# Mattdl/CLsurvey

Hardware: AMD Instinct MI355X
Metric: images/sec (train+importance pass), EWC small_VGG9 Tiny-ImageNet task batch (higher is better)
Workload: dtype f32 (bf16x6 split operands on the conv fwd/bwd-data matrix products, fp32 accumulate); 1 GPU; EWC small_VGG9_cl_128_128, Tiny-ImageNet shapes (3x64x64, 20 classes), batch 200: train step + Fisher step (BASELINE configs[1]); batch=200, parallelism=1 GPU

## Files before the change

clsurvey_amd/csrc/bsconv.hip:

```cpp
#include "common.hpp"
#include "bs_weight.hpp"
#include "wgrad_reduce.hpp"
#include <cstdlib>

#ifndef BS_ABL
#define BS_ABL 0
#endif

namespace {

constexpr int BS_WT_JOBS = 24;
struct BsWtJobs { int n; int pad; clhip_wino_wt j[BS_WT_JOBS]; int first[BS_WT_JOBS + 1]; };

__global__ __launch_bounds__(256) void bs_weight_multi_kernel(BsWtJobs J) {
    int jb = 0;
    for (int i = 1; i < J.n; ++i) jb = ((int)blockIdx.x >= J.first[i]) ? i : jb;
    bs_weight_block(J.j[jb], (int)blockIdx.x - J.first[jb], (int)threadIdx.x);
}

template <int RW_, int RH_, int NI_, int WAVES_M_, int WM_, int WN_, int KS_ = 3>
struct BsGeo {
    static constexpr int RW = RW_, RH = RH_, NI = NI_, WAVES_M = WAVES_M_, WAVES_N = 4 / WAVES_M_, WM = WM_, WN = WN_;
    static constexpr int KS = KS_, HP = KS_ / 2, TAPS = KS_ * KS_;
    static constexpr int BM = RW * RH * NI;
    static_assert(BM == 32 * WAVES_M * WM, "pixels per block = M tiles of the waves");
    static_assert(32 * WAVES_N * WN == BS_BN, "64 output channels per block");
    static constexpr int MTW = RW >= 16 ? 16 : 8, MTH = 32 / MTW;
    static_assert(RW % MTW == 0 && RH % MTH == 0, "whole M tiles");
    static constexpr int MT_PER_ROW = RW / MTW, MT_PER_IMG = MT_PER_ROW * (RH / MTH);
    static constexpr int IPR = RW == 8 ? 2 : 1;
    static_assert(NI % IPR == 0, "image pairs");
    static constexpr int HW_ = RW + 2 * HP, HR = RH + 2 * HP;
    static constexpr int P = (IPR * HW_ + 7) / 16 * 16 + 8;
    static_assert(P >= IPR * HW_ && P % 16 == 8, "pitch");
    static constexpr int ROWS = (NI / IPR) * HR;
    static constexpr int PLANE_SLOTS = (ROWS - 1) * P + IPR * HW_;
    static constexpr int PLANE_BYTES = PLANE_SLOTS * 16;
    static constexpr int BUF_BYTES = 6 * PLANE_BYTES;
    static constexpr int NHALO = NI * HR * HW_;
    static constexpr int ITEMS = 2 * NHALO;
    static constexpr int ROUNDS = (ITEMS + 255) / 256;
    static_assert(ROUNDS * 256 - ITEMS <= ITEMS, "the last round wraps at most once");
    static constexpr int TPR = WM < MT_PER_ROW ? WM : MT_PER_ROW;
    static_assert(WM % TPR == 0 && MT_PER_ROW % TPR == 0 && MT_PER_IMG % WM == 0, "a wave's tiles form a rectangle inside one image");
    static constexpr int RGW = TPR * MTW, RGH = 32 * WM / RGW;
    static constexpr int TS = 32 * WM + 4;
    static_assert(4 * 32 * TS * 4 <= 2 * BUF_BYTES, "transposition buffers fit the staging LDS");
};

template <class G, int MODE, bool UNPOOL>
__device__ __forceinline__ void bs_conv_body(
    unsigned char* __restrict__ lds, const int b, const float* __restrict__ in, const clhip_u32x4* __restrict__ wimg,
    const float* __restrict__ bias, const float* __restrict__ mask_src, float* __restrict__ out, uint8_t* __restrict__ pool_idx, int N,
    int Cin, int Cout, int H, int W, int relu, int tiles_x, int tiles_y, int npb) {
    constexpr int RW = G::RW, RH = G::RH, NI = G::NI, WM = G::WM, WN = G::WN, P = G::P, HR = G::HR, HW_ = G::HW_;
    constexpr int ROUNDS = G::ROUNDS;

    const int tid = threadIdx.x, lane = tid & 63, wave = tid >> 6;
    const int kts = (Cout + BS_BN - 1) / BS_BN;
    const int kt = (b >> 3) % kts, pb = (b / (8 * kts)) * 8 + (b & 7);
    if (pb >= npb) return;
    const int tx = pb % tiles_x, ty = (pb / tiles_x) % tiles_y, grp = pb / (tiles_x * tiles_y);
    const int n0 = grp * NI, y0 = ty * RH, x0 = tx * RW;
    const int n_chunks = Cin / BS_CK;
    const int IH = UNPOOL ? H >> 1 : H, IW = UNPOOL ? W >> 1 : W;
    const int plane_in = IH * IW;

    const float* in_blk = in + (size_t)n0 * Cin * plane_in;
    const __amdgpu_buffer_rsrc_t rs_x = clhip_rsrc(in_blk, (size_t)(N - n0) * Cin * plane_in * sizeof(float));
    const __amdgpu_buffer_rsrc_t rs_i = clhip_rsrc(UNPOOL ? pool_idx + (size_t)n0 * Cin * plane_in : pool_idx,
                                                   UNPOOL ? (size_t)(N - n0) * Cin * plane_in : 0);
    const int n_nt = (Cout + 31) / 32;
    constexpr int TAPS = G::TAPS, KS = G::KS;
    const __amdgpu_buffer_rsrc_t rs_w = clhip_rsrc(wimg, (size_t)n_nt * n_chunks * 3 * TAPS * 1024);

    int xoff[ROUNDS], lw[ROUNDS], pos[ROUNDS];
#pragma unroll
    for (int r = 0; r < ROUNDS; ++r) {
        const int it_ = r * 256 + tid, it = it_ < G::ITEMS ? it_ : it_ - G::ITEMS;
        const int h = it >= G::NHALO ? 1 : 0, p = it - h * G::NHALO;
        const int ni = p / (HR * HW_), rem = p - ni * (HR * HW_), hy = rem / HW_, hx = rem - hy * HW_;
        const int gy = y0 + hy - G::HP, gx = x0 + hx - G::HP, n = n0 + ni;
        const bool ok = n < N && gy >= 0 && gy < H && gx >= 0 && gx < W;
        const int e = UNPOOL ? (gy >> 1) * IW + (gx >> 1) : gy * IW + gx;
        xoff[r] = ok ? (ni * Cin + 8 * h) * plane_in + e : CLHIP_OOB;
        pos[r] = ((gy & 1) << 1) | (gx & 1);
        lw[r] = (h * G::PLANE_SLOTS + ((ni / G::IPR) * HR + hy) * P + (ni % G::IPR) * HW_ + hx) * 16;
    }
    float xr[ROUNDS][8];
    unsigned xi[UNPOOL ? ROUNDS : 1][8];
    auto load_chunk = [&](int c) {
        if (BS_ABL & 8) return;
        const int cb = c * BS_CK * plane_in;
#pragma unroll
        for (int r = 0; r < ROUNDS; ++r)
#pragma unroll
            for (int e = 0; e < 8; ++e) {
                const int so = cb + e * plane_in;
                xr[r][e] = clhip_buf_load(rs_x, xoff[r] != CLHIP_OOB ? xoff[r] * 4 : CLHIP_OOB, so * 4);
                if constexpr (UNPOOL) xi[r][e] = clhip_buf_load_u8(rs_i, xoff[r], so);
            }
    };
    auto store_chunk = [&](int buf) {
        if (BS_ABL & 4) return;
#pragma unroll
        for (int r = 0; r < ROUNDS; ++r) {
            float v[8];
#pragma unroll
            for (int e = 0; e < 8; ++e) {
                if constexpr (UNPOOL) v[e] = xi[r][e] == (unsigned)pos[r] ? xr[r][e] : 0.f;
                else v[e] = xr[r][e];
            }
            clhip_u32x4 q0, q1, q2;
            bs_split8(v, q0, q1, q2);
            unsigned char* d = lds + buf * G::BUF_BYTES + lw[r];
            *reinterpret_cast<clhip_u32x4*>(d) = q0;
            *reinterpret_cast<clhip_u32x4*>(d + 2 * G::PLANE_BYTES) = q1;
            *reinterpret_cast<clhip_u32x4*>(d + 4 * G::PLANE_BYTES) = q2;
        }
    };

    const int wm = wave % G::WAVES_M, wn = wave / G::WAVES_M;
    const int m = lane & 31, kh = lane >> 5;
    const int mw = m >> 2, mq = m & 3;
    const int prow = 2 * (mw / (G::MTW / 2)) + (mq >> 1), pcol = 2 * (mw % (G::MTW / 2)) + (mq & 1);
    int abase[WM];
#pragma unroll
    for (int i = 0; i < WM; ++i) {
        const int mt = wm * WM + i;
        const int ni = mt / G::MT_PER_IMG, rem = mt - ni * G::MT_PER_IMG, tr = rem / G::MT_PER_ROW, tc = rem - tr * G::MT_PER_ROW;
        abase[i] = (kh * G::PLANE_SLOTS + ((ni / G::IPR) * HR + tr * G::MTH + prow) * P + (ni % G::IPR) * HW_ + tc * G::MTW + pcol) * 16;
    }
    const int nt0 = kt * (BS_BN / 32) + wn * WN;
    int wvoff[WN];
#pragma unroll
    for (int j = 0; j < WN; ++j) wvoff[j] = (nt0 + j < n_nt) ? ((nt0 + j) * n_chunks * 3 * TAPS * 64 + lane) * 16 : CLHIP_OOB;
    auto load_b = [&](clhip_u32x4 (&bq)[WN][3], int c, int tap) {
        if (BS_ABL & 2) return;
        const int so = (c * 3 * TAPS + tap * 3) * 1024;
#pragma unroll
        for (int j = 0; j < WN; ++j)
#pragma unroll
            for (int s = 0; s < 3; ++s) bq[j][s] = __builtin_amdgcn_raw_buffer_load_b128(rs_w, wvoff[j], so + s * 1024, 0);
    };

    floatx16 acc[WM][WN], accl[WM][WN];
#pragma unroll
    for (int i = 0; i < WM; ++i)
#pragma unroll
        for (int j = 0; j < WN; ++j)
#pragma unroll
            for (int r = 0; r < 16; ++r) {
// ... 186 lines not shown
                    }
                }
                if (!ok || ((BS_ABL & 16) && y00 != 12345.678f)) continue;
                const size_t o = ((size_t)n * Cout + k) * chw + (size_t)oh * W + ow;
                if (odd) {
                    const bool row1 = oh + 1 < H, col1 = ow + 1 < W;
                    if (MODE == 1 && mask_src) {
                        y00 = mask_src[o] > 0.f ? y00 : 0.f;
                        if (col1) y01 = mask_src[o + 1] > 0.f ? y01 : 0.f;
                        if (row1) y10 = mask_src[o + W] > 0.f ? y10 : 0.f;
                        if (row1 && col1) y11 = mask_src[o + W + 1] > 0.f ? y11 : 0.f;
                    }
                    out[o] = y00;
                    if (col1) out[o + 1] = y01;
                    if (row1) out[o + W] = y10;
                    if (row1 && col1) out[o + W + 1] = y11;
                } else {
                    if (MODE == 1 && mask_src) {
                        const float2 m0 = *reinterpret_cast<const float2*>(mask_src + o), m1 = *reinterpret_cast<const float2*>(mask_src + o + W);
                        y00 = m0.x > 0.f ? y00 : 0.f; y01 = m0.y > 0.f ? y01 : 0.f;
                        y10 = m1.x > 0.f ? y10 : 0.f; y11 = m1.y > 0.f ? y11 : 0.f;
                    }
                    *reinterpret_cast<float2*>(out + o) = make_float2(y00, y01);
                    *reinterpret_cast<float2*>(out + o + W) = make_float2(y10, y11);
                }
            }
        }
    }
    }
}

template <class G, bool UNPOOL>
constexpr int bs_blocks_per_cu() {
    return (3 * 2 * G::BUF_BYTES <= 160 * 1024 && (G::RW == 32 || (!UNPOOL && G::KS == 3))) ? 3 : 2;
}

template <class G, int MODE, bool UNPOOL>
__global__ __launch_bounds__(256, (bs_blocks_per_cu<G, UNPOOL>())) void bs_conv_kernel(
    const float* __restrict__ in, const clhip_u32x4* __restrict__ wimg, const float* __restrict__ bias,
    const float* __restrict__ mask_src, float* __restrict__ out, uint8_t* __restrict__ pool_idx, int N, int Cin, int Cout, int H,
    int W, int relu, int tiles_x, int tiles_y, int npb) {
    __shared__ __attribute__((aligned(16))) unsigned char lds[2 * G::BUF_BYTES];
    bs_conv_body<G, MODE, UNPOOL>(lds, (int)blockIdx.x, in, wimg, bias, mask_src, out, pool_idx, N, Cin, Cout, H, W, relu, tiles_x, tiles_y, npb);
}

template <class GA, class GB, int MODE, bool UNPOOL>
__global__ __launch_bounds__(256, (bs_blocks_per_cu<GA, UNPOOL>() < bs_blocks_per_cu<GB, UNPOOL>() ? bs_blocks_per_cu<GA, UNPOOL>()
                                                                                                  : bs_blocks_per_cu<GB, UNPOOL>()))
void bs_conv_mixed_kernel(const float* __restrict__ in, const clhip_u32x4* __restrict__ wimg, const float* __restrict__ bias,
                          const float* __restrict__ mask_src, float* __restrict__ out, uint8_t* __restrict__ pool_idx, int N, int Cin,
                          int Cout, int H, int W, int relu, int blocks_a, int NA, int tiles_xa, int tiles_ya, int npb_a, int tiles_xb,
                          int tiles_yb, int npb_b) {
    constexpr int LB = 2 * (GA::BUF_BYTES > GB::BUF_BYTES ? GA::BUF_BYTES : GB::BUF_BYTES);
    __shared__ __attribute__((aligned(16))) unsigned char lds[LB];
    const int b = (int)blockIdx.x;
    if (b < blocks_a) {
        bs_conv_body<GA, MODE, UNPOOL>(lds, b, in, wimg, bias, mask_src, out, pool_idx, NA, Cin, Cout, H, W, relu, tiles_xa, tiles_ya, npb_a);
    } else {
        const size_t in_img = (size_t)Cin * (UNPOOL ? (size_t)(H >> 1) * (W >> 1) : (size_t)H * W);
        const bool pool = MODE == 0 && pool_idx != nullptr;
        const size_t out_img = (size_t)Cout * (pool ? (size_t)(H >> 1) * (W >> 1) : (size_t)H * W);
        uint8_t* idx_b = pool_idx ? pool_idx + (size_t)NA * (UNPOOL ? in_img : out_img) : nullptr;
        bs_conv_body<GB, MODE, UNPOOL>(lds, b - blocks_a, in + (size_t)NA * in_img, wimg, bias,
                                       mask_src ? mask_src + (size_t)NA * Cout * H * W : nullptr, out + (size_t)NA * out_img, idx_b, N - NA,
                                       Cin, Cout, H, W, relu, tiles_xb, tiles_yb, npb_b);
    }
}
// ... 134 lines not shown
BsMixed bs_one_geo(int N, int Cout, int H, int W) {
    BsMixed m{};
    m.txa = (W + G::RW - 1) / G::RW; m.tya = (H + G::RH - 1) / G::RH; m.NA = N;
    const long long npb = (long long)m.txa * m.tya * ((N + G::NI - 1) / G::NI);
    const long long blocks = (npb + 7) / 8 * 8 * ((Cout + BS_BN - 1) / BS_BN);
    m.blocks = (npb > 0x7fffffffLL || blocks > 0x7fffffffLL) ? 0 : blocks;
    m.npb_a = (int)npb; m.blocks_a = (int)m.blocks;
    return m;
}

template <bool UNPOOL>
int bs_launch_riders(const float* in, const clhip_u32x4* wimg, const float* mask_src, float* out, uint8_t* pool_idx, int N, int Cin,
                     int Cout, int H, int W, const RedJobs& jobs, int place, int riders, hipStream_t s) {
#define BS_RIDE(GA_, GB_, M_) return bs_launch_riders_geo<GA_, GB_, UNPOOL>(in, wimg, mask_src, out, pool_idx, N, Cin, Cout, H, W, M_, jobs, place, riders, s)
    if (W > 16 && !((H | W) & 1)) {
        BsMixed m;
        if (bs_mixed32_plan<UNPOOL>(N, Cout, H, W, m)) BS_RIDE(BsGA32, BsGB32, m);
    }
    using G16 = BsGeo<16, 8, 1, 2, 2, 1>;
    using G8 = BsGeo<8, 8, 2, 2, 2, 1>;
    if (W > 16) BS_RIDE(BsGA32, BsGA32, bs_one_geo<BsGA32>(N, Cout, H, W));
    if (W > 8) BS_RIDE(G16, G16, bs_one_geo<G16>(N, Cout, H, W));
    BS_RIDE(G8, G8, bs_one_geo<G8>(N, Cout, H, W));
#undef BS_RIDE
}

template <int MODE>
int bs_launch5(const float* in, const clhip_u32x4* wimg, const float* bias, const float* mask_src, float* out, int N, int Cin, int Cout,
               int H, int W, int relu, hipStream_t s) {
    if (W > 16) return bs_launch_geo<BsGeo<32, 4, 1, 2, 2, 1, 5>, MODE, false>(in, wimg, bias, mask_src, out, nullptr, N, Cin, Cout, H, W, relu, s);
    return bs_launch_geo<BsGeo<16, 8, 1, 2, 2, 1, 5>, MODE, false>(in, wimg, bias, mask_src, out, nullptr, N, Cin, Cout, H, W, relu, s);
}

}

bool clhip_internal_bs_ok(int Cin, int Cout, int H, int W) {
    return Cin >= 32 && Cin % 32 == 0 && Cout >= 64 && Cout % 64 == 0 && H >= 4 && W >= 4;
}

bool clhip_internal_bs_index_ok(int Cin, int Cout, int H, int W, int ks) {
    const long long px = (long long)H * W, ni = (ks == 3 && W <= 8) ? 2 : 1;
    const long long img = (long long)((Cout + 31) / 32) * ((Cin + BS_CK - 1) / BS_CK) * 3 * ks * ks * 1024;
    return ni * Cin * px < (1LL << 29) && Cout * px < (1LL << 29) && img <= 0x7fffffffLL;
}

bool clhip_internal_bs_preferred(int Cin, int Cout, int H, int W) {
    static const int mode = bs_env_int("CLHIP_BS", 1);
    if (mode == 0 || !clhip_internal_bs_ok(Cin, Cout, H, W)) return false;
    if (mode == 2) return true;
    const long long px = (long long)H * W;
    return (px >= 1024 && px <= 4096 && Cin <= 128 && Cout <= 128) || (px >= 512 && px < 1024 && Cin >= 256 && Cout >= 256);
}
bool clhip_internal_bs5_preferred(int Cin, int Cout, int H, int W) {
    static const int mode = bs_env_int("CLHIP_BS", 1);
    return mode != 0 && clhip_internal_bs_ok(Cin, Cout, H, W) && W > 8;
}

size_t clhip_internal_bs_ws(int Cin, int Cout) {
    return (size_t)((Cout + 31) / 32) * ((Cin + BS_CK - 1) / BS_CK) * 27 * 1024;
}
size_t clhip_internal_bs5_ws(int Cin, int Cout) {
    return (size_t)((Cout + 31) / 32) * ((Cin + BS_CK - 1) / BS_CK) * 75 * 1024;
}

int clhip_internal_bs_weights(const clhip_wino_wt* jobs, int n, hipStream_t s) {
    if (n <= 0) return 0;
// ... 110 lines not shown
    if (N <= 0 || !clhip_internal_bs_ok(K, C, H, W)) return CLHIP_ENOTSUP;
    if (!dy || !w || !dx || !ws || ws_bytes < clhip_internal_bs_ws(K, C)) return CLHIP_EINVAL;
    if (!clhip_internal_bs_index_ok(K, C, H, W, 3)) return CLHIP_EINVAL;
    if (((H | W) & 1) && idx_u8_or_null) return CLHIP_ENOTSUP;
    const clhip_wino_wt job{w, static_cast<float*>(ws), C, K, 1, 0};
    const int rc = clhip_internal_bs_weights(&job, 1, as_stream(stream));
    if (rc) return rc;
    return clhip_internal_bs_conv_u(1, dy, ws, nullptr, relu_src, dx, const_cast<uint8_t*>(idx_u8_or_null), idx_u8_or_null != nullptr,
                                    N, K, C, H, W, 0, as_stream(stream));
}

int clhip_conv3x3_bs_bwd_data_riders(const float* dy, const uint8_t* idx_u8_or_null, const float* w, const float* relu_src, float* dx, int N,
                                     int C, int K, int H, int W, void* ws, size_t ws_bytes, const clhip_reduce_job* jobs, int n_jobs,
                                     int place, int riders, void* stream) {
    if (N <= 0 || !clhip_internal_bs_ok(K, C, H, W)) return CLHIP_ENOTSUP;
    if (!dy || !w || !dx || !ws || ws_bytes < clhip_internal_bs_ws(K, C)) return CLHIP_EINVAL;
    if (!clhip_internal_bs_index_ok(K, C, H, W, 3)) return CLHIP_EINVAL;
    if (((H | W) & 1) && idx_u8_or_null) return CLHIP_ENOTSUP;
    if (!jobs || n_jobs < 1 || n_jobs > CLHIP_WGRAD_JOBS_MAX || place < 1 || place > 3 || riders < 8 || riders % 8 || riders > (1 << 20))
        return CLHIP_ENOTSUP;
    clhip_wgrad_job q[CLHIP_WGRAD_JOBS_MAX];
    for (int i = 0; i < n_jobs; ++i) {
        const clhip_reduce_job& j = jobs[i];
        if (!j.slabs || !j.dw || j.K <= 0 || j.C <= 0 || j.splits <= 0 || (j.taps != 9 && j.taps != 25)) return CLHIP_EINVAL;
        q[i] = clhip_wgrad_job{j.slabs, j.dw, j.db, j.K, j.C, j.splits, j.taps};
    }
    const clhip_wino_wt job{w, static_cast<float*>(ws), C, K, 1, 0};
    const int rc = clhip_internal_bs_weights(&job, 1, as_stream(stream));
    if (rc) return rc;
    return clhip_internal_bs_conv_u_riders(dy, ws, relu_src, dx, const_cast<uint8_t*>(idx_u8_or_null), idx_u8_or_null != nullptr, N, K, C, H,
                                           W, q, n_jobs, place, riders, as_stream(stream));
}

}
```

clsurvey_amd/csrc/wino.hip:

```cpp
#include "common.hpp"
#include "weight_images.hpp"
#include <cstdlib>

namespace {


struct WGeoW {
    static constexpr int TCB = 4, TRB = 4, NIMG = 4;
    static constexpr int PW = 2 * TCB + 2;
    static constexpr int PR = 2 * TRB + 2;
    static constexpr int PLANE = NIMG * PR * PW;
    static constexpr int X_FLOATS = WCK * PLANE;
    static constexpr int BUF = W_FLOATS + X_FLOATS;
};

__global__ __launch_bounds__(256) void wino_weight_kernel(const float* __restrict__ w, float* __restrict__ U, int Ko, int Ci,
                                                          int mode, int n_chunks) {
    const int total = ((Ko + WKT - 1) / WKT) * n_chunks * WCK * WKT;
    for (int i = blockIdx.x * 256 + threadIdx.x; i < total; i += gridDim.x * 256) {
        const int k_l = i % WKT, c_l = (i / WKT) % WCK, chunk = (i / (WKT * WCK)) % n_chunks, kt = i / (WKT * WCK * n_chunks);
        const int k = kt * WKT + k_l, c = chunk * WCK + c_l;
        float g[3][3];
#pragma unroll
        for (int r = 0; r < 3; ++r)
#pragma unroll
            for (int s = 0; s < 3; ++s) {
                float v = 0.f;
                if (k < Ko && c < Ci)
                    v = mode == 0 ? w[((size_t)k * Ci + c) * 9 + r * 3 + s]
                                  : w[((size_t)c * Ko + k) * 9 + (2 - r) * 3 + (2 - s)];
                g[r][s] = v;
            }
        float t[4][3];
#pragma unroll
// ... 565 lines not shown
__device__ __forceinline__ void wino_conv16_body(
    float* __restrict__ lds, const int bid,
    const float* __restrict__ in, const float* __restrict__ U, const float* __restrict__ bias,
    const float* __restrict__ mask_src, float* __restrict__ out, uint8_t* __restrict__ pool_idx,
    int N, int Cin, int Cout, int relu) {
    constexpr int H = 8, W = 8, NIMG = KT2;
    constexpr int PW = 10, PR = 10, PLANE = NIMG * PR * PW;
    constexpr bool ADIRECT = wino16_adirect<UNPOOL, KT2>;
    constexpr int WOFF = ADIRECT ? 0 : W_FLOATS;
    constexpr int X_FLOATS = WCK * PLANE, BUF = WOFF + X_FLOATS;
    static_assert(wino16_lds_floats<UNPOOL, KT2>() == 2 * BUF + WKT, "LDS size of the wrappers");
    float* const bias_s = lds + 2 * BUF;
    const int tid = threadIdx.x, lane = tid & 63, wave = tid >> 6;
    const int wk = KT2 == 2 ? wave & 1 : wave, wp = KT2 == 2 ? wave >> 1 : 0;
    constexpr int KW = 16 * KT2;
    const int ti = lane & 15, q = lane >> 4;
    const int n_grp = (N + NIMG - 1) / NIMG;
    const int kt = bid / n_grp, ng = bid - kt * n_grp;
    const int n0 = ng * NIMG, ko0 = kt * WKT;
    const int n_chunks = (Cin + WCK - 1) / WCK;
    if (MODE == 0 && tid < WKT) bias_s[tid] = (bias && ko0 + tid < Cout) ? bias[ko0 + tid] : 0.f;

    constexpr int Hi = UNPOOL ? H >> 1 : H, Wi = UNPOOL ? W >> 1 : W;
    constexpr int plane_in = Hi * Wi;
    const float* in_blk = in + (size_t)n0 * Cin * plane_in;
    const __amdgpu_buffer_rsrc_t rs_x = clhip_rsrc(in_blk, (size_t)(N - n0) * Cin * plane_in * sizeof(float));
    const __amdgpu_buffer_rsrc_t rs_i = clhip_rsrc(UNPOOL ? pool_idx + (size_t)n0 * Cin * plane_in : pool_idx,
                                                   UNPOOL ? (size_t)(N - n0) * Cin * plane_in : 0);
    const __amdgpu_buffer_rsrc_t rs_u = ADIRECT
        ? clhip_rsrc(U + (size_t)((Cout + WKT - 1) / WKT) * n_chunks * W_FLOATS + (size_t)kt * 2 * n_chunks * WD_FLOATS,
                     (size_t)2 * n_chunks * WD_FLOATS * sizeof(float))
        : clhip_rsrc(U + (size_t)kt * n_chunks * W_FLOATS, (size_t)n_chunks * W_FLOATS * sizeof(float));

    constexpr int W_IT = ADIRECT ? 0 : W_FLOATS / 4 / 256;
    constexpr int X_IT = (X_FLOATS + 255) / 256;
    constexpr int NU = W_IT + X_IT;
    float4 wv[W_IT ? W_IT : 1];
    float xr[X_IT];
    unsigned xi[UNPOOL ? X_IT : 1];
    int xoff[X_IT], xcode[UNPOOL ? X_IT : 1];
#pragma unroll
    for (int j = 0; j < X_IT; ++j) {
        const int e = tid + 256 * j;
        xoff[j] = CLHIP_OOB;
        if (e < X_FLOATS) {
            const int cl = e / PLANE, rem = e - cl * PLANE;
            const int col = rem % PW, rr = rem / PW;
            const int row = rr % PR, nb = rr / PR;
            const int h = row - 1, w = col - 1;
            if (n0 + nb < N && h >= 0 && h < H && w >= 0 && w < W) {
                if constexpr (UNPOOL) {
                    xoff[j] = (nb * Cin + cl) * plane_in + (h >> 1) * Wi + (w >> 1);
                    xcode[j] = ((h & 1) << 1) | (w & 1);
                } else {
                    xoff[j] = ((nb * Cin + cl) * plane_in + h * W + w) * 4;
                }
            }
        }
    }
    auto load_unit = [&](int u, int chunk) {
        const int cw = chunk < n_chunks ? chunk : n_chunks - 1;
        if (u < W_IT) {
            wv[u] = clhip_buf_load4(rs_u, (tid + 256 * u) * 16, cw * W_FLOATS * 4);
        } else {
            const int j = u - W_IT;
            const int xb = cw * WCK * plane_in;
            if constexpr (UNPOOL) {
                xr[j] = clhip_buf_load(rs_x, xoff[j] != CLHIP_OOB ? xoff[j] * 4 : CLHIP_OOB, xb * 4);
                xi[j] = clhip_buf_load_u8(rs_i, xoff[j], xb);
            } else {
                xr[j] = clhip_buf_load(rs_x, xoff[j], xb * 4);
            }
        }
    };
    auto store_unit = [&](int u, int bo) {
        if (u < W_IT) {
            float* wd = lds + bo + 4 * (tid + 256 * u);
            *reinterpret_cast<floatx4*>(wd) = floatx4{wv[u].x, wv[u].y, wv[u].z, wv[u].w};
        } else {
            const int j = u - W_IT;
            float* xs = lds + bo + WOFF;
            if (256 * (j + 1) <= X_FLOATS || tid + 256 * j < X_FLOATS) {
                if constexpr (UNPOOL) xs[tid + 256 * j] = ((int)xi[j] == xcode[j]) ? xr[j] : 0.f;
                else xs[tid + 256 * j] = xr[j];
            }
        }
    };

    const int t_row = ti >> 2, t_col = ti & 3;
    const int d_off = WOFF + q * PLANE + (wp * PR + 2 * t_row) * PW + 2 * t_col;
    const int a_off = (q * WKT + wk * KW + ti) * WFP;

    floatx4v acc[KT2][16];
#pragma unroll
    for (int k2 = 0; k2 < KT2; ++k2)
#pragma unroll
        for (int f = 0; f < 16; ++f) acc[k2][f] = floatx4v{0.f, 0.f, 0.f, 0.f};

    typedef float f2 __attribute__((ext_vector_type(2)));
    constexpr int NQ = WCK / 4;
    floatx4 av[2][KT2][4];
    float vv[2][16];
    f2 dlo[4], dhi[4], tlo[4], thi[4];
    auto rd_a = [&](const float* abase, int quad, int k2, int fq, int slot, int c4) {
        if constexpr (ADIRECT) {
            const int cc = c4 < 2 * n_chunks ? c4 : 2 * n_chunks - 1;
            const clhip_u32x4 v = __builtin_amdgcn_raw_buffer_load_b128(rs_u, (((wk * KW) >> 4) + k2) * 4096 + fq * 1024 + lane * 16,
                                                                        cc * (WD_FLOATS * 4), 0);
            av[slot][k2][fq] = floatx4{__uint_as_float(v.x), __uint_as_float(v.y), __uint_as_float(v.z), __uint_as_float(v.w)};
        } else {
            av[slot][k2][fq] = *reinterpret_cast<const floatx4*>(abase + 4 * quad * WKT * WFP + k2 * 16 * WFP + 4 * fq);
        }
    };
    auto rd_d = [&](const float* dbase, int quad, int r) {
        dlo[r] = *reinterpret_cast<const f2*>(dbase + 4 * quad * PLANE + r * PW);
        dhi[r] = *reinterpret_cast<const f2*>(dbase + 4 * quad * PLANE + r * PW + 2);
    };
// ... 136 lines not shown
__device__ __forceinline__ void wino_conv16g_body(
    float* __restrict__ lds, const int bid,
    const float* __restrict__ in, const float* __restrict__ U, const float* __restrict__ bias,
    const float* __restrict__ mask_src, float* __restrict__ out, uint8_t* __restrict__ pool_idx,
    int N, int Cin, int Cout, int H, int W, int relu, int tiles_w, int tiles_h, int n_pix_blocks) {
    static_assert(TC * TR == 16, "16 tiles per wave");
    constexpr int CQ = 4;
    constexpr int NE = 2 * TR / EROWS;
    static_assert(NE * EROWS == 2 * TR && (NE == 1 || !UNPOOL || EROWS == 4), "whole entities");
    constexpr int PW = 2 * TC + 2, PRE = 2 * EROWS + 2, PLANE = NE * PRE * PW;
    constexpr int X_FLOATS = CQ * PLANE, BUF = X_FLOATS;
    static_assert(wino16g_lds_floats<TC, TR, EROWS>() == 2 * BUF + WKT, "LDS size of the wrappers");
    float* const bias_s = lds + 2 * BUF;
    const int tid = threadIdx.x, lane = tid & 63, wave = tid >> 6;
    const int wk = wave & 1, wp = wave >> 1;
    const int ti = lane & 15, q = lane >> 4;
    const int kt = bid / n_pix_blocks, pb = bid - kt * n_pix_blocks;
    const int bw = pb % tiles_w, v0 = (pb / tiles_w) * NE;
    const int nb0 = v0 / tiles_h, w0 = bw * 2 * TC;
    const int ko0 = kt * WKT;
    const int n_chunks = Cin / CQ;
    if (MODE == 0 && tid < WKT) bias_s[tid] = (bias && ko0 + tid < Cout) ? bias[ko0 + tid] : 0.f;

    const int Hi = UNPOOL ? H >> 1 : H, Wi = UNPOOL ? W >> 1 : W;
    const int plane_in = Hi * Wi;
    const float* in_img = in + (size_t)nb0 * Cin * plane_in;
    const __amdgpu_buffer_rsrc_t rs_x = clhip_rsrc(in_img, (size_t)(N - nb0) * Cin * plane_in * sizeof(float));
    const __amdgpu_buffer_rsrc_t rs_i = clhip_rsrc(UNPOOL ? pool_idx + (size_t)nb0 * Cin * plane_in : pool_idx,
                                                   UNPOOL ? (size_t)(N - nb0) * Cin * plane_in : 0);
    const __amdgpu_buffer_rsrc_t rs_u =
        clhip_rsrc(U + (size_t)((Cout + WKT - 1) / WKT) * (Cin / WCK) * W_FLOATS + (size_t)kt * n_chunks * WD_FLOATS,
                   (size_t)n_chunks * WD_FLOATS * sizeof(float));

    constexpr int X_IT = (X_FLOATS + 255) / 256;
    struct Stage {
        float4 wv[1];
        float xr[X_IT];
        unsigned xi[UNPOOL ? X_IT : 1];
    };
    int xoff[X_IT], xcode[UNPOOL ? X_IT : 1];
#pragma unroll
    for (int j = 0; j < X_IT; ++j) {
        const int e = tid + 256 * j;
        xoff[j] = CLHIP_OOB;
        if (e < X_FLOATS) {
            const int cl = e / PLANE, rem = e - cl * PLANE;
            const int col = rem % PW, rr = rem / PW;
            const int row = rr % PRE, v = v0 + rr / PRE;
            const int nn = v / tiles_h, g = v - nn * tiles_h;
            const int h = g * 2 * EROWS - 1 + row, w = w0 - 1 + col;
            if (nn < N && h >= 0 && h < H && w >= 0 && w < W) {
                if constexpr (UNPOOL) {
                    xoff[j] = ((nn - nb0) * Cin + cl) * plane_in + (h >> 1) * Wi + (w >> 1);
                    xcode[j] = ((h & 1) << 1) | (w & 1);
                } else {
                    xoff[j] = (((nn - nb0) * Cin + cl) * plane_in + h * W + w) * 4;
                }
            }
        }
    }
    auto load_chunk = [&](int chunk, Stage& st) {
        const int cw = chunk < n_chunks ? chunk : n_chunks - 1;
        const int xb = cw * CQ * plane_in;
#pragma unroll
        for (int j = 0; j < X_IT; ++j) {
            if constexpr (UNPOOL) {
                st.xr[j] = clhip_buf_load(rs_x, xoff[j] != CLHIP_OOB ? xoff[j] * 4 : CLHIP_OOB, xb * 4);
                st.xi[j] = clhip_buf_load_u8(rs_i, xoff[j], xb);
            } else {
                st.xr[j] = clhip_buf_load(rs_x, xoff[j], xb * 4);
            }
        }
    };
    auto store_chunk = [&](int bo, const Stage& st) {
        float* xs = lds + bo;
#pragma unroll
        for (int j = 0; j < X_IT; ++j)
            if (256 * (j + 1) <= X_FLOATS || tid + 256 * j < X_FLOATS) {
                if constexpr (UNPOOL) xs[tid + 256 * j] = ((int)st.xi[j] == xcode[j]) ? st.xr[j] : 0.f;
                else xs[tid + 256 * j] = st.xr[j];
            }
    };

    const int t_rowb = wp * TR + ti / TC, t_col = ti % TC;
    const int t_ent = t_rowb / EROWS, t_row = t_rowb % EROWS;
    const int d_off = q * PLANE + (t_ent * PRE + 2 * t_row) * PW + 2 * t_col;
    const int a_off = (q * WKT + wk * 32 + ti) * WFP;

    floatx4v acc[2][16];
#pragma unroll
    for (int k2 = 0; k2 < 2; ++k2)
#pragma unroll
        for (int f = 0; f < 16; ++f) acc[k2][f] = floatx4v{0.f, 0.f, 0.f, 0.f};

    typedef float f2 __attribute__((ext_vector_type(2)));
    struct AReg { floatx4 a0[4], a1[4]; };
    const int a_voff = wk * (2 * 4 * 256 * 4) + lane * 16;
    auto load_a = [&](int chunk, AReg& A) {
        const int ca = (chunk < n_chunks ? chunk : n_chunks - 1) * (WD_FLOATS * 4);
#pragma unroll
        for (int fq = 0; fq < 4; ++fq) {
            const clhip_u32x4 v0 = __builtin_amdgcn_raw_buffer_load_b128(rs_u, a_voff + fq * 1024, ca, 0);
            const clhip_u32x4 v1 = __builtin_amdgcn_raw_buffer_load_b128(rs_u, a_voff + 4096 + fq * 1024, ca, 0);
            A.a0[fq] = floatx4{__uint_as_float(v0.x), __uint_as_float(v0.y), __uint_as_float(v0.z), __uint_as_float(v0.w)};
            A.a1[fq] = floatx4{__uint_as_float(v1.x), __uint_as_float(v1.y), __uint_as_float(v1.z), __uint_as_float(v1.w)};
        }
    };
    auto compute = [&](int bo, const AReg& A) {
        const float* ab = lds + bo + a_off; (void)ab;
        const float* db = lds + bo + d_off;
        f2 dlo[4], dhi[4];
#pragma unroll
        for (int r = 0; r < 4; ++r) {
// ... 488 lines not shown
            hipLaunchKernelGGL((wino_conv16_kernel<MODE, UNPOOL, 1>), dim3((unsigned)blocks), dim3(256), 0, s, in, U, bias, mask_src, out,
                               pool_idx, N, Cin, Cout, relu);
        else
            hipLaunchKernelGGL((wino_conv16_kernel<MODE, UNPOOL, 2>), dim3((unsigned)blocks), dim3(256), 0, s, in, U, bias, mask_src, out,
                               pool_idx, N, Cin, Cout, relu);
        CLHIP_LAUNCH_CHECK();
        return 0;
    }
#define WINO_16G(TC_, TR_, ER_, UNP_)                                                                                          \
    do {                                                                                                                       \
        const int tiles_w = ((W + 1) / 2 + TC_ - 1) / TC_, groups = ((H + 1) / 2 + ER_ - 1) / ER_;                              \
        constexpr int NE_ = 2 * TR_ / ER_;                                                                                      \
        const long long npb = (((long long)N * groups + NE_ - 1) / NE_) * tiles_w, blocks = npb * kts;                          \
        if (blocks <= 0 || blocks > 0x7fffffffLL) return CLHIP_EINVAL;                                                          \
        hipLaunchKernelGGL((wino_conv16g_kernel<TC_, TR_, ER_, MODE, UNP_>), dim3((unsigned)blocks), dim3(256), 0, s, in, U,    \
                           bias, mask_src, out, pool_idx, N, Cin, Cout, H, W, relu, tiles_w, groups, (int)npb);                 \
        CLHIP_LAUNCH_CHECK();                                                                                                   \
        return 0;                                                                                                               \
    } while (0)
    if ((H | W) & 1) { if (W <= 16) WINO_16G(8, 2, 1, false); }
    else if (W >= 16) WINO_16G(8, 2, 4, UNPOOL);
    else if (H == 8 && W == 8) WINO_16G(4, 4, 4, UNPOOL);
#undef WINO_16G
    using G = WGeoW;
    const int tiles_w = ((W + 1) / 2 + G::TCB - 1) / G::TCB, tiles_h = ((H + 1) / 2 + G::TRB - 1) / G::TRB, ngrp = (N + G::NIMG - 1) / G::NIMG;
    const long long npb = (long long)tiles_w * tiles_h * ngrp, blocks = npb * kts;
    if (blocks <= 0 || blocks > 0x7fffffffLL) return CLHIP_EINVAL;
    hipLaunchKernelGGL((wino_conv_kernel<MODE, UNPOOL>), dim3((unsigned)blocks), dim3(256), 0, s, in, U, bias, mask_src, out, pool_idx,
                       N, Cin, Cout, H, W, relu, tiles_w, tiles_h, (int)npb);
    CLHIP_LAUNCH_CHECK();
    return 0;
}

}

bool clhip_internal_wino_ok(int Cin, int Cout, int H, int W) {
    if (Cin % WCK || Cin < 16 || Cout % 32 || H < 4 || W < 8) return false;
    if (((H | W) & 1) == 0) return true;
    return W > 8 && W <= 16;
}

size_t clhip_internal_wino_ws(int Cin, int Cout) {
    return (size_t)((Cout + WKT - 1) / WKT) * ((Cin + WCK - 1) / WCK) * WU_FLOATS * sizeof(float);
}

int clhip_internal_wino_conv_u(int mode, const float* in, const float* U, const float* bias, const float* mask_src, float* out,
                               uint8_t* pool_idx, int unpool, int N, int Cin, int Cout, int H, int W, int relu, hipStream_t s) {
    if (!in || !U || !out || !clhip_internal_wino_ok(Cin, Cout, H, W)) return CLHIP_EINVAL;
    if (((H | W) & 1) && (pool_idx || unpool)) return CLHIP_ENOTSUP;
    if (mode == 0) return launch_wino<0, false>(in, U, bias, nullptr, out, pool_idx, N, Cin, Cout, H, W, relu, s);
    if (unpool) return launch_wino<1, true>(in, U, nullptr, mask_src, out, pool_idx, N, Cin, Cout, H, W, 0, s);
    return launch_wino<1, false>(in, U, nullptr, mask_src, out, nullptr, N, Cin, Cout, H, W, 0, s);
}

int clhip_internal_wino_weights(const clhip_wino_wt* jobs, int n, hipStream_t s) {
    if (n <= 0) return 0;
    if (!jobs) return CLHIP_EINVAL;
    for (int base = 0; base < n; base += WT_JOBS) {
        WtJobs J;
        J.n = n - base < WT_JOBS ? n - base : WT_JOBS;
        J.pad = 0;
        int blocks = 0;
        for (int i = 0; i < J.n; ++i) {
            const clhip_wino_wt& q = jobs[base + i];
            if (!q.w || !q.U || q.Ko <= 0 || q.Ci <= 0) return CLHIP_EINVAL;
            J.j[i] = q;
// ... 245 lines not shown
```

Baseline: 302,800 images/s.

## Stage unpooled inputs once per pooling window and vectorize plain 8x8 staging

The unpool path of the bs conv now loads each pooled source element once and writes it to both horizontally adjacent LDS slots, roughly halving staging items. It also lifts the 3-blocks-per-CU occupancy limit for unpool kernels. The wino16g unpool path scatters one load to a 2x2 window of four slots, and the plain 8x8 wino path uses float4 loads with a halo ring zeroed once. A host-side stage-map export is added for verification, and the new index maps carry some correctness risk at edges and in the spare-thread writes.

```diff
diff --git a/clsurvey_amd/csrc/bsconv.hip b/clsurvey_amd/csrc/bsconv.hip
--- a/clsurvey_amd/csrc/bsconv.hip
+++ b/clsurvey_amd/csrc/bsconv.hip
@@ -1,6 +1,7 @@
 #include "common.hpp"
 #include "bs_weight.hpp"
 #include "wgrad_reduce.hpp"
+#include "stage_map.hpp"
 #include <cstdlib>
 
 #ifndef BS_ABL
@@ -53,15 +54,16 @@
     unsigned char* __restrict__ lds, const int b, const float* __restrict__ in, const clhip_u32x4* __restrict__ wimg,
     const float* __restrict__ bias, const float* __restrict__ mask_src, float* __restrict__ out, uint8_t* __restrict__ pool_idx, int N,
     int Cin, int Cout, int H, int W, int relu, int tiles_x, int tiles_y, int npb) {
-    constexpr int RW = G::RW, RH = G::RH, NI = G::NI, WM = G::WM, WN = G::WN, P = G::P, HR = G::HR, HW_ = G::HW_;
-    constexpr int ROUNDS = G::ROUNDS;
+    constexpr int WM = G::WM, WN = G::WN, P = G::P, HR = G::HR, HW_ = G::HW_;
+    using UM = BsUnpoolMap<G>;
+    constexpr int ROUNDS = UNPOOL ? UM::ROUNDS : G::ROUNDS, PX = UNPOOL ? 2 : 1;
 
     const int tid = threadIdx.x, lane = tid & 63, wave = tid >> 6;
     const int kts = (Cout + BS_BN - 1) / BS_BN;
     const int kt = (b >> 3) % kts, pb = (b / (8 * kts)) * 8 + (b & 7);
     if (pb >= npb) return;
-    const int tx = pb % tiles_x, ty = (pb / tiles_x) % tiles_y, grp = pb / (tiles_x * tiles_y);
-    const int n0 = grp * NI, y0 = ty * RH, x0 = tx * RW;
+    int n0, y0, x0;
+    bs_tile_origin<G>(pb, tiles_x, tiles_y, n0, y0, x0);
     const int n_chunks = Cin / BS_CK;
     const int IH = UNPOOL ? H >> 1 : H, IW = UNPOOL ? W >> 1 : W;
     const int plane_in = IH * IW;
@@ -74,18 +76,29 @@
     constexpr int TAPS = G::TAPS, KS = G::KS;
     const __amdgpu_buffer_rsrc_t rs_w = clhip_rsrc(wimg, (size_t)n_nt * n_chunks * 3 * TAPS * 1024);
 
-    int xoff[ROUNDS], lw[ROUNDS], pos[ROUNDS];
+    int xoff[ROUNDS], lw[ROUNDS][PX], pos[ROUNDS][PX];
 #pragma unroll
     for (int r = 0; r < ROUNDS; ++r) {
-        const int it_ = r * 256 + tid, it = it_ < G::ITEMS ? it_ : it_ - G::ITEMS;
-        const int h = it >= G::NHALO ? 1 : 0, p = it - h * G::NHALO;
-        const int ni = p / (HR * HW_), rem = p - ni * (HR * HW_), hy = rem / HW_, hx = rem - hy * HW_;
-        const int gy = y0 + hy - G::HP, gx = x0 + hx - G::HP, n = n0 + ni;
-        const bool ok = n < N && gy >= 0 && gy < H && gx >= 0 && gx < W;
-        const int e = UNPOOL ? (gy >> 1) * IW + (gx >> 1) : gy * IW + gx;
-        xoff[r] = ok ? (ni * Cin + 8 * h) * plane_in + e : CLHIP_OOB;
-        pos[r] = ((gy & 1) << 1) | (gx & 1);
-        lw[r] = (h * G::PLANE_SLOTS + ((ni / G::IPR) * HR + hy) * P + (ni % G::IPR) * HW_ + hx) * 16;
+        if constexpr (UNPOOL) {
+            const BsStageItem s = UM::item(r * 256 + tid);
+            int ps[2];
+            const int so = bs_unpool_source<G>(s, n0, y0, x0, N, Cin, H, W, ps);
+            xoff[r] = so >= 0 ? so : CLHIP_OOB;
+#pragma unroll
+            for (int p = 0; p < PX; ++p) {
+                pos[r][p] = ps[p];
+                lw[r][p] = UM::slot(s, p) * 16;
+            }
+        } else {
+            const int it_ = r * 256 + tid, it = it_ < G::ITEMS ? it_ : it_ - G::ITEMS;
+            const int h = it >= G::NHALO ? 1 : 0, p = it - h * G::NHALO;
+            const int ni = p / (HR * HW_), rem = p - ni * (HR * HW_), hy = rem / HW_, hx = rem - hy * HW_;
+            const int gy = y0 + hy - G::HP, gx = x0 + hx - G::HP, n = n0 + ni;
+            const bool ok = n < N && gy >= 0 && gy < H && gx >= 0 && gx < W;
+            xoff[r] = ok ? (ni * Cin + 8 * h) * plane_in + gy * IW + gx : CLHIP_OOB;
+            pos[r][0] = 0;
+            lw[r][0] = (h * G::PLANE_SLOTS + ((ni / G::IPR) * HR + hy) * P + (ni % G::IPR) * HW_ + hx) * 16;
+        }
     }
     float xr[ROUNDS][8];
     unsigned xi[UNPOOL ? ROUNDS : 1][8];
@@ -104,20 +117,22 @@
     auto store_chunk = [&](int buf) {
         if (BS_ABL & 4) return;
 #pragma unroll
-        for (int r = 0; r < ROUNDS; ++r) {
-            float v[8];
-#pragma unroll
-            for (int e = 0; e < 8; ++e) {
-                if constexpr (UNPOOL) v[e] = xi[r][e] == (unsigned)pos[r] ? xr[r][e] : 0.f;
-                else v[e] = xr[r][e];
+        for (int r = 0; r < ROUNDS; ++r)
+#pragma unroll
+            for (int p = 0; p < PX; ++p) {
+                float v[8];
+#pragma unroll
+                for (int e = 0; e < 8; ++e) {
+                    if constexpr (UNPOOL) v[e] = xi[r][e] == (unsigned)pos[r][p] ? xr[r][e] : 0.f;
+                    else v[e] = xr[r][e];
+                }
+                clhip_u32x4 q0, q1, q2;
+                bs_split8(v, q0, q1, q2);
+                unsigned char* d = lds + buf * G::BUF_BYTES + lw[r][p];
+                *reinterpret_cast<clhip_u32x4*>(d) = q0;
+                *reinterpret_cast<clhip_u32x4*>(d + 2 * G::PLANE_BYTES) = q1;
+                *reinterpret_cast<clhip_u32x4*>(d + 4 * G::PLANE_BYTES) = q2;
             }
-            clhip_u32x4 q0, q1, q2;
-            bs_split8(v, q0, q1, q2);
-            unsigned char* d = lds + buf * G::BUF_BYTES + lw[r];
-            *reinterpret_cast<clhip_u32x4*>(d) = q0;
-            *reinterpret_cast<clhip_u32x4*>(d + 2 * G::PLANE_BYTES) = q1;
-            *reinterpret_cast<clhip_u32x4*>(d + 4 * G::PLANE_BYTES) = q2;
-        }
     };
 
     const int wm = wave % G::WAVES_M, wn = wave / G::WAVES_M;
@@ -370,7 +385,7 @@
 
 template <class G, bool UNPOOL>
 constexpr int bs_blocks_per_cu() {
-    return (3 * 2 * G::BUF_BYTES <= 160 * 1024 && (G::RW == 32 || (!UNPOOL && G::KS == 3))) ? 3 : 2;
+    return (3 * 2 * G::BUF_BYTES <= 160 * 1024 && (G::RW == 32 || G::KS == 3)) ? 3 : 2;
 }
 
 template <class G, int MODE, bool UNPOOL>
@@ -571,6 +586,31 @@
     return bs_launch_geo<BsGeo<16, 8, 1, 2, 2, 1, 5>, MODE, false>(in, wimg, bias, mask_src, out, nullptr, N, Cin, Cout, H, W, relu, s);
 }
 
+template <class G>
+int bs_stage_map(int N, int Cin, int H, int W, int block, int* src, int* pos, int* slot, int cap) {
+    using UM = BsUnpoolMap<G>;
+    const int tiles_x = (W + G::RW - 1) / G::RW, tiles_y = (H + G::RH - 1) / G::RH, groups = (N + G::NI - 1) / G::NI;
+    const long long npb = (long long)tiles_x * tiles_y * groups;
+    if (npb > 0x7fffffffLL) return CLHIP_EINVAL;
+    if (block < 0) return (int)npb;
+    if (block >= npb || !src || !pos || !slot) return CLHIP_EINVAL;
+    int n0, y0, x0, n = 0;
+    bs_tile_origin<G>(block, tiles_x, tiles_y, n0, y0, x0);
+    const int plane_in = (H >> 1) * (W >> 1);
+    for (int it = 0; it < UM::ROUNDS * 256; ++it) {
+        const BsStageItem s = UM::item(it);
+        int ps[2];
+        const int so = bs_unpool_source<G>(s, n0, y0, x0, N, Cin, H, W, ps);
+        for (int p = 0; p < 2; ++p, ++n) {
+            if (n >= cap) continue;
+            src[n] = so >= 0 ? n0 * Cin * plane_in + so : -1;
+            pos[n] = ps[p];
+            slot[n] = UM::slot(s, p);
+        }
+    }
+    return n;
+}
+
 }
 
 bool clhip_internal_bs_ok(int Cin, int Cout, int H, int W) {
@@ -747,4 +787,19 @@
                                            W, q, n_jobs, place, riders, as_stream(stream));
 }
 
-}
+int clhip_internal_stage_map(int kernel, int geo, int N, int Cin, int H, int W, int block, int* src, int* pos, int* slot, int cap) {
+    if (kernel < 0 || kernel > 2) return CLHIP_ENOTSUP;
+    if (N <= 0 || Cin <= 0 || H < 2 || W < 2 || ((H | W) & 1) || cap < 0) return CLHIP_EINVAL;
+    if ((long long)N * Cin * (H >> 1) * (W >> 1) > 0x7fffffffLL) return CLHIP_EINVAL;
+    if (kernel >= 1) return clhip_internal_wino_stage_map(kernel, geo, N, Cin, H, W, block, src, pos, slot, cap);
+    if (Cin < BS_CK || Cin % BS_CK) return CLHIP_EINVAL;
+    switch (geo) {
+        case 0: return bs_stage_map<BsGA32>(N, Cin, H, W, block, src, pos, slot, cap);
+        case 1: return bs_stage_map<BsGB32>(N, Cin, H, W, block, src, pos, slot, cap);
+        case 2: return bs_stage_map<BsGeo<16, 8, 1, 2, 2, 1>>(N, Cin, H, W, block, src, pos, slot, cap);
+        case 3: return bs_stage_map<BsGeo<8, 8, 2, 2, 2, 1>>(N, Cin, H, W, block, src, pos, slot, cap);
+    }
+    return CLHIP_ENOTSUP;
+}
+
+}
diff --git a/clsurvey_amd/csrc/stage_map.hpp b/clsurvey_amd/csrc/stage_map.hpp
--- /dev/null
+++ b/clsurvey_amd/csrc/stage_map.hpp
@@ -0,0 +1,115 @@
+#pragma once
+
+struct BsStageItem {
+    int ni, h, hy;
+    int hx[2];
+    int spare;
+};
+
+template <class G>
+struct BsUnpoolMap {
+    static constexpr int WO = G::HP & 1;
+    static constexpr int NWC = (G::HW_ + WO + 1) / 2;
+    static constexpr int NWIN = G::NI * G::HR * NWC;
+    static constexpr int ITEMS = 2 * NWIN;
+    static constexpr int ROUNDS = (ITEMS + 255) / 256;
+    static_assert(G::RW % 2 == 0 && G::HW_ % 2 == 0, "tiles start and end on window boundaries");
+    static constexpr int PAD = G::P - G::IPR * G::HW_;
+    static_assert(PAD >= 1 && G::ROWS >= 2, "somewhere for the spare threads to write");
+
+    __host__ __device__ static BsStageItem item(int it) {
+        BsStageItem s;
+        s.spare = it - ITEMS;
+        if (it >= ITEMS) it = 0;
+        s.h = it >= NWIN ? 1 : 0;
+        const int p = it - s.h * NWIN;
+        s.ni = p / (G::HR * NWC);
+        const int rem = p - s.ni * (G::HR * NWC);
+        s.hy = rem / NWC;
+        const int wc = rem - s.hy * NWC, a = 2 * wc - WO;
+        s.hx[0] = a < 0 ? 0 : a;
+        s.hx[1] = a + 1 > G::HW_ - 1 ? G::HW_ - 1 : a + 1;
+        return s;
+    }
+    __host__ __device__ static int slot(int h, int ni, int hy, int hx) {
+        return h * G::PLANE_SLOTS + ((ni / G::IPR) * G::HR + hy) * G::P + (ni % G::IPR) * G::HW_ + hx;
+    }
+    __host__ __device__ static int slot(const BsStageItem& s, int p) {
+        if (s.spare >= 0) return (s.spare / PAD) % (G::ROWS - 1) * G::P + G::IPR * G::HW_ + s.spare % PAD;
+        return slot(s.h, s.ni, s.hy, s.hx[p]);
+    }
+};
+
+template <class G>
+__host__ __device__ inline int bs_unpool_source(const BsStageItem& s, int n0, int y0, int x0, int N, int Cin, int H, int W, int (&pos)[2]) {
+    const int gy = y0 + s.hy - G::HP, gx = x0 + s.hx[0] - G::HP;
+    pos[0] = ((gy & 1) << 1) | (gx & 1);
+    pos[1] = ((gy & 1) << 1) | ((x0 + s.hx[1] - G::HP) & 1);
+    const bool ok = s.spare < 0 && n0 + s.ni < N && gy >= 0 && gy < H && gx >= 0 && gx < W;
+    return ok ? (s.ni * Cin + 8 * s.h) * ((H >> 1) * (W >> 1)) + (gy >> 1) * (W >> 1) + (gx >> 1) : -1;
+}
+
+template <class G>
+__host__ __device__ inline void bs_tile_origin(int pb, int tiles_x, int tiles_y, int& n0, int& y0, int& x0) {
+    const int tx = pb % tiles_x, ty = (pb / tiles_x) % tiles_y, grp = pb / (tiles_x * tiles_y);
+    n0 = grp * G::NI; y0 = ty * G::RH; x0 = tx * G::RW;
+}
+
+struct W16gStageItem {
+    int cl, ent, wr, wc;
+    int idx[4], pos[4];
+};
+
+template <int TC, int TR, int EROWS>
+struct W16gUnpoolMap {
+    static constexpr int CQ = 4, NE = 2 * TR / EROWS, PW = 2 * TC + 2, PRE = 2 * EROWS + 2, PLANE = NE * PRE * PW;
+    static constexpr int NWR = EROWS + 2, NWC = TC + 2, ITEMS = CQ * NE * NWR * NWC, ROUNDS = (ITEMS + 255) / 256;
+
+    __host__ __device__ static W16gStageItem item(int e) {
+        W16gStageItem s;
+        s.cl = e / (NE * NWR * NWC);
+        int rem = e - s.cl * (NE * NWR * NWC);
+        s.ent = rem / (NWR * NWC);
+        rem -= s.ent * (NWR * NWC);
+        s.wr = rem / NWC;
+        s.wc = rem - s.wr * NWC;
+        for (int p = 0; p < 4; ++p) {
+            int row = 2 * s.wr - 1 + (p >> 1), col = 2 * s.wc - 1 + (p & 1);
+            row = row < 0 ? 0 : row > PRE - 1 ? PRE - 1 : row;
+            col = col < 0 ? 0 : col > PW - 1 ? PW - 1 : col;
+            s.idx[p] = s.cl * PLANE + (s.ent * PRE + row) * PW + col;
+            s.pos[p] = (((row + 1) & 1) << 1) | ((col + 1) & 1);
+        }
+        return s;
+    }
+    __host__ __device__ static int source(const W16gStageItem& s, int v0, int w0, int tiles_h, int N, int Cin, int H, int W) {
+        const int Hi = H >> 1, Wi = W >> 1, v = v0 + s.ent, nn = v / tiles_h, g = v - nn * tiles_h;
+        const int ph = g * EROWS + s.wr - 1, pw = (w0 >> 1) + s.wc - 1;
+        const bool ok = nn < N && ph >= 0 && ph < Hi && pw >= 0 && pw < Wi;
+        return ok ? ((nn - v0 / tiles_h) * Cin + s.cl) * (Hi * Wi) + ph * Wi + pw : -1;
+    }
+};
+
+template <int KT2>
+struct W16PlainMap {
+    static constexpr int NIMG = KT2, CK = 8, PW = 10, PR = 10, PLANE = NIMG * PR * PW;
+    static constexpr int ITEMS = CK * NIMG * 16;
+    static constexpr int RING = CK * NIMG * 36;
+    static_assert(ITEMS <= 256, "one item per thread");
+    __host__ __device__ static void item(int f, int Cin, int& nb, int& src, int& idx) {
+        const int cl = f / (NIMG * 16), rem = f - cl * (NIMG * 16);
+        nb = rem >> 4;
+        const int row = (rem & 15) >> 1, half = rem & 1;
+        src = (nb * Cin + cl) * 64 + row * 8 + half * 4;
+        idx = cl * PLANE + (nb * PR + row + 1) * PW + 1 + half * 4;
+    }
+    __host__ __device__ static int ring(int r) {
+        const int pl = r / 36, k = r - pl * 36;
+        const int row = k < 10 ? 0 : k < 20 ? 9 : 1 + ((k - 20) >> 1), col = k < 10 ? k : k < 20 ? k - 10 : ((k - 20) & 1) * 9;
+        return pl * (PR * PW) + row * PW + col;
+    }
+};
+
+extern "C" __attribute__((visibility("default"))) int clhip_internal_stage_map(int kernel, int geo, int N, int Cin, int H, int W, int block, int* src, int* pos, int* slot, int cap);
+
+int clhip_internal_wino_stage_map(int kernel, int geo, int N, int Cin, int H, int W, int block, int* src, int* pos, int* slot, int cap);
diff --git a/clsurvey_amd/csrc/wino.hip b/clsurvey_amd/csrc/wino.hip
--- a/clsurvey_amd/csrc/wino.hip
+++ b/clsurvey_amd/csrc/wino.hip
@@ -1,5 +1,6 @@
 #include "common.hpp"
 #include "weight_images.hpp"
+#include "stage_map.hpp"
 #include <cstdlib>
 
 namespace {
@@ -631,15 +632,34 @@
                      (size_t)2 * n_chunks * WD_FLOATS * sizeof(float))
         : clhip_rsrc(U + (size_t)kt * n_chunks * W_FLOATS, (size_t)n_chunks * W_FLOATS * sizeof(float));
 
+    constexpr bool VEC = !UNPOOL;
+    using PM = W16PlainMap<KT2>;
+    static_assert(PM::PLANE == PLANE && PM::CK == WCK, "stage_map.hpp states this kernel's chunk buffer");
     constexpr int W_IT = ADIRECT ? 0 : W_FLOATS / 4 / 256;
-    constexpr int X_IT = (X_FLOATS + 255) / 256;
+    constexpr int X_IT = VEC ? 1 : (X_FLOATS + 255) / 256;
     constexpr int NU = W_IT + X_IT;
     float4 wv[W_IT ? W_IT : 1];
+    float4 xv = make_float4(0.f, 0.f, 0.f, 0.f);
     float xr[X_IT];
     unsigned xi[UNPOOL ? X_IT : 1];
     int xoff[X_IT], xcode[UNPOOL ? X_IT : 1];
-#pragma unroll
-    for (int j = 0; j < X_IT; ++j) {
+    int xvi = 0;
+    if constexpr (VEC) {
+        int nb, src;
+        PM::item(tid < PM::ITEMS ? tid : 0, Cin, nb, src, xvi);
+        xoff[0] = (tid < PM::ITEMS && n0 + nb < N) ? src * 4 : CLHIP_OOB;
+#pragma unroll
+        for (int j = 0; j < (PM::RING + 255) / 256; ++j) {
+            const int r = tid + 256 * j;
+            if (256 * (j + 1) <= PM::RING || r < PM::RING) {
+                const int o = WOFF + PM::ring(r);
+                lds[o] = 0.f;
+                lds[BUF + o] = 0.f;
+            }
+        }
+    }
+#pragma unroll
+    for (int j = 0; j < (VEC ? 0 : X_IT); ++j) {
         const int e = tid + 256 * j;
         xoff[j] = CLHIP_OOB;
         if (e < X_FLOATS) {
@@ -668,7 +688,7 @@
                 xr[j] = clhip_buf_load(rs_x, xoff[j] != CLHIP_OOB ? xoff[j] * 4 : CLHIP_OOB, xb * 4);
                 xi[j] = clhip_buf_load_u8(rs_i, xoff[j], xb);
             } else {
-                xr[j] = clhip_buf_load(rs_x, xoff[j], xb * 4);
+                xv = clhip_buf_load4(rs_x, xoff[0], xb * 4);
             }
         }
     };
@@ -679,9 +699,12 @@
         } else {
             const int j = u - W_IT;
             float* xs = lds + bo + WOFF;
-            if (256 * (j + 1) <= X_FLOATS || tid + 256 * j < X_FLOATS) {
-                if constexpr (UNPOOL) xs[tid + 256 * j] = ((int)xi[j] == xcode[j]) ? xr[j] : 0.f;
-                else xs[tid + 256 * j] = xr[j];
+            if constexpr (VEC) {
+                if (PM::ITEMS == 256 || tid < PM::ITEMS) {
+                    xs[xvi] = xv.x; xs[xvi + 1] = xv.y; xs[xvi + 2] = xv.z; xs[xvi + 3] = xv.w;
+                }
+            } else if (256 * (j + 1) <= X_FLOATS || tid + 256 * j < X_FLOATS) {
+                xs[tid + 256 * j] = ((int)xi[j] == xcode[j]) ? xr[j] : 0.f;
             }
         }
     };
@@ -884,31 +907,34 @@
         clhip_rsrc(U + (size_t)((Cout + WKT - 1) / WKT) * (Cin / WCK) * W_FLOATS + (size_t)kt * n_chunks * WD_FLOATS,
                    (size_t)n_chunks * WD_FLOATS * sizeof(float));
 
-    constexpr int X_IT = (X_FLOATS + 255) / 256;
+    using UM = W16gUnpoolMap<TC, TR, EROWS>;
+    static_assert(UM::PLANE == PLANE && UM::PW == PW && UM::PRE == PRE, "stage_map.hpp states this kernel's chunk buffer");
+    constexpr int X_ITEMS = UNPOOL ? UM::ITEMS : X_FLOATS;
+    constexpr int X_IT = (X_ITEMS + 255) / 256;
     struct Stage {
         float4 wv[1];
         float xr[X_IT];
         unsigned xi[UNPOOL ? X_IT : 1];
     };
-    int xoff[X_IT], xcode[UNPOOL ? X_IT : 1];
+    int xoff[X_IT];
+    int xa[UNPOOL ? X_IT : 1][4], xp[UNPOOL ? X_IT : 1][4];
 #pragma unroll
     for (int j = 0; j < X_IT; ++j) {
         const int e = tid + 256 * j;
         xoff[j] = CLHIP_OOB;
-        if (e < X_FLOATS) {
+        if constexpr (UNPOOL) {
+            const W16gStageItem it = UM::item(e < X_ITEMS ? e : 0);
+            const int so = UM::source(it, v0, w0, tiles_h, N, Cin, H, W);
+            if (e < X_ITEMS && so >= 0) xoff[j] = so;
+#pragma unroll
+            for (int p = 0; p < 4; ++p) { xa[j][p] = it.idx[p]; xp[j][p] = it.pos[p]; }
+        } else if (e < X_FLOATS) {
             const int cl = e / PLANE, rem = e - cl * PLANE;
             const int col = rem % PW, rr = rem / PW;
             const int row = rr % PRE, v = v0 + rr / PRE;
             const int nn = v / tiles_h, g = v - nn * tiles_h;
             const int h = g * 2 * EROWS - 1 + row, w = w0 - 1 + col;
-            if (nn < N && h >= 0 && h < H && w >= 0 && w < W) {
-                if constexpr (UNPOOL) {
-                    xoff[j] = ((nn - nb0) * Cin + cl) * plane_in + (h >> 1) * Wi + (w >> 1);
-                    xcode[j] = ((h & 1) << 1) | (w & 1);
-                } else {
-                    xoff[j] = (((nn - nb0) * Cin + cl) * plane_in + h * W + w) * 4;
-                }
-            }
+            if (nn < N && h >= 0 && h < H && w >= 0 && w < W) xoff[j] = (((nn - nb0) * Cin + cl) * plane_in + h * W + w) * 4;
         }
     }
     auto load_chunk = [&](int chunk, Stage& st) {
@@ -928,9 +954,11 @@
         float* xs = lds + bo;
 #pragma unroll
         for (int j = 0; j < X_IT; ++j)
-            if (256 * (j + 1) <= X_FLOATS || tid + 256 * j < X_FLOATS) {
-                if constexpr (UNPOOL) xs[tid + 256 * j] = ((int)st.xi[j] == xcode[j]) ? st.xr[j] : 0.f;
-                else xs[tid + 256 * j] = st.xr[j];
+            if (256 * (j + 1) <= X_ITEMS || tid + 256 * j < X_ITEMS) {
+                if constexpr (UNPOOL) {
+#pragma unroll
+                    for (int p = 0; p < 4; ++p) xs[xa[j][p]] = ((int)st.xi[j] == xp[j][p]) ? st.xr[j] : 0.f;
+                } else xs[tid + 256 * j] = st.xr[j];
             }
     };
 
@@ -1485,6 +1513,60 @@
     return 0;
 }
 
+template <int TC, int TR, int EROWS>
+int wino16g_stage_map(int N, int Cin, int H, int W, int block, int* src, int* pos, int* slot, int cap) {
+    using UM = W16gUnpoolMap<TC, TR, EROWS>;
+    const int tiles_w = ((W + 1) / 2 + TC - 1) / TC, tiles_h = ((H + 1) / 2 + EROWS - 1) / EROWS;
+    const long long npb = (((long long)N * tiles_h + UM::NE - 1) / UM::NE) * tiles_w;
+    if (npb > 0x7fffffffLL) return CLHIP_EINVAL;
+    if (block < 0) return (int)npb;
+    if (block >= npb || !src || !pos || !slot) return CLHIP_EINVAL;
+    const int bw = block % tiles_w, v0 = (block / tiles_w) * UM::NE, nb0 = v0 / tiles_h, w0 = bw * 2 * TC;
+    int n = 0;
+    for (int e = 0; e < UM::ITEMS; ++e) {
+        const W16gStageItem it = UM::item(e);
+        const int so = UM::source(it, v0, w0, tiles_h, N, Cin, H, W);
+        for (int p = 0; p < 4; ++p, ++n) {
+            if (n >= cap) continue;
+            src[n] = so >= 0 ? nb0 * Cin * (H >> 1) * (W >> 1) + so : -1;
+            pos[n] = it.pos[p];
+            slot[n] = it.idx[p];
+        }
+    }
+    return n;
+}
+
+}
+
+template <int KT2>
+static int wino16_plain_stage_map(int N, int Cin, int block, int* src, int* pos, int* slot, int cap) {
+    using PM = W16PlainMap<KT2>;
+    const int n_grp = (N + KT2 - 1) / KT2;
+    if (block < 0) return n_grp;
+    if (block >= n_grp || !src || !pos || !slot) return CLHIP_EINVAL;
+    const int n0 = block * KT2;
+    int n = 0;
+    auto put = [&](int s_, int q) { if (n < cap) { src[n] = s_; pos[n] = -1; slot[n] = q; } ++n; };
+    for (int f = 0; f < PM::ITEMS; ++f) {
+        int nb, so, idx;
+        PM::item(f, Cin, nb, so, idx);
+        for (int e = 0; e < 4; ++e) put(n0 + nb < N ? n0 * Cin * 64 + so + e : -1, idx + e);
+    }
+    for (int r = 0; r < PM::RING; ++r) put(-1, PM::ring(r));
+    return n;
+}
+
+int clhip_internal_wino_stage_map(int kernel, int geo, int N, int Cin, int H, int W, int block, int* src, int* pos, int* slot, int cap) {
+    if (Cin % WCK || Cin < 16) return CLHIP_EINVAL;
+    if (kernel == 2) {
+        if (H != 8 || W != 8) return CLHIP_EINVAL;
+        if (geo == 0) return wino16_plain_stage_map<1>(N, Cin, block, src, pos, slot, cap);
+        if (geo == 1) return wino16_plain_stage_map<2>(N, Cin, block, src, pos, slot, cap);
+        return CLHIP_ENOTSUP;
+    }
+    if (geo == 0) return wino16g_stage_map<8, 2, 4>(N, Cin, H, W, block, src, pos, slot, cap);
+    if (geo == 1) return wino16g_stage_map<4, 4, 4>(N, Cin, H, W, block, src, pos, slot, cap);
+    return CLHIP_ENOTSUP;
 }
 
 bool clhip_internal_wino_ok(int Cin, int Cout, int H, int W) {
```

Result: faster. 308,100 images/s (median of 6 runs) (+1.7%).
